# PABannier/bark.cpp

Hardware: NVIDIA H100
Metric: audio sec/sec (inverse RTF), bark-small f16, batch 1 per GPU, semantic->coarse->fine->encodec (higher is better)
Workload: dtype f16 weights/operands, f32 accumulate (reference arithmetic)

## Files before the change

bark.cpp_b200/csrc/bark_api.cu:

```cuda
#include "../../include/bark_b200.h"
#include "context.h"
#include "codec_kernels.h"
#include "gpt_kernels.h"

#include <algorithm>
#include <cmath>
#include <cstring>
#include <stdexcept>

using namespace bark;

namespace {

thread_local int g_device_override = -1;
bool quiet() { static const bool q = [] { const char * e = getenv("BARK_B200_QUIET"); return e && *e && *e != '0'; }(); return q; }

inline bool is_alpha(unsigned char c) { return (c >= 'a' && c <= 'z') || (c >= 'A' && c <= 'Z'); }
inline bool is_digit(unsigned char c) { return c >= '0' && c <= '9'; }
inline bool is_punct(unsigned char c) { return c > 32 && c < 127 && !is_alpha(c) && !is_digit(c); }

char fold_accent(unsigned char second) {
    const unsigned cp = 0xC0u + (second - 0x80u);
    const bool lower = cp >= 0xE0;
    const unsigned up = lower ? cp - 0x20 : cp;
// ... 626 lines not shown
}

extern "C" struct bark_context * bark_load_model(const char * model_path, struct bark_context_params params, uint32_t seed) {
    const int64_t t0 = now_us();
    if (!model_path) { fprintf(stderr, "%s: null model path\n", __func__); return nullptr; }
    cudaDeviceProp prop;
    const int dev = select_device(__func__, &prop);
    if (dev < 0) return nullptr;
    bark_context * ctx = new bark_context();
    ctx->device = dev;
    ctx->n_sm = ctx->n_sm_total = prop.multiProcessorCount;
    if (ctx->n_sm >= 132) ctx->n_sm = 128;
    { const char * e = getenv("BARK_B200_MODE"); ctx->fast_mode = e && !strcmp(e, "fast"); }
    { const char * e = getenv("BARK_B200_DECODE_CTAS"); if (e && atoi(e) >= 64 && atoi(e) <= ctx->n_sm) ctx->n_sm = atoi(e); }
    { const char * e = getenv("BARK_B200_SAMPLE_FLAG_EVERY"); ctx->debug_flag_every = e ? atoi(e) : 0; }
    { const char * e = getenv("BARK_B200_KV_REUSE"); ctx->kv_reuse = !(e && !strcmp(e, "0")); }
    { const char * e = getenv("BARK_B200_DECODE"); ctx->use_decode_kernel = !(e && !strcmp(e, "multi")); }
    { const char * e = getenv("BARK_B200_DECODE_TIMING_TID"); if (e && atoi(e) >= 0 && atoi(e) < 512) ctx->timing_tid = atoi(e) & ~31; }
    { const char * e = getenv("BARK_B200_POLL_NS"); if (e && atoi(e) >= 0 && atoi(e) <= 100000) ctx->poll_ns = (unsigned) atoi(e); }
    { const char * e = getenv("BARK_B200_HEADSTART"); if (e) { unsigned v[6]; if (sscanf(e, "%u:%u:%u:%u:%u:%u", &v[0], &v[1], &v[2], &v[3], &v[4], &v[5]) == 6) for (int i = 0; i < 6; i++) ctx->headstart[i] = std::min(v[i], 100000u); } }
    ctx->params = params;
    const bool loaded = guarded(false, [&] {
    BARK_CUDA_CHECK(cudaStreamCreateWithFlags(&ctx->stream, cudaStreamNonBlocking));
    if (!load_model_file(model_path, ctx)) return false;
    alloc_workspace(ctx);
    { const char * e = getenv("BARK_B200_TAG_BASE"); if (e) ctx->tag_base = (unsigned) strtoul(e, nullptr, 0); }
    if (getenv("BARK_B200_DECODE_TIMING")) { ctx->d_timing = (unsigned long long *) ctx_alloc(ctx, 256 * 32 * 8); BARK_CUDA_CHECK(cudaMemset(ctx->d_timing, 0, 256 * 32 * 8)); }
    BARK_CUDA_CHECK(cudaStreamSynchronize(ctx->stream));
    return true;
    });
// ... 262 lines not shown
```

bark.cpp_b200/csrc/common.cuh:

```cuda
#pragma once

#include <cuda_fp16.h>
#include <cuda_runtime.h>
#include <atomic>
#include <exception>
#include <stdexcept>
#include <stdint.h>
#include <stdio.h>
#include <stdlib.h>

namespace bark { struct CudaFailure { cudaError_t err; const char * file; int line; }; }
#define BARK_CUDA_CHECK(expr)                                                                         \
    do {                                                                                              \
        cudaError_t err__ = (expr);                                                                   \
        if (err__ != cudaSuccess) {                                                                   \
            fprintf(stderr, "bark_b200: CUDA error %s at %s:%d: %s\n", cudaGetErrorName(err__), __FILE__, __LINE__, \
                    cudaGetErrorString(err__));                                                       \
            throw ::bark::CudaFailure{err__, __FILE__, __LINE__};                                     \
        }                                                                                             \
    } while (0)

namespace bark {

template <typename R, typename F> inline R guarded(R fail, F && f) {
// ... 1 lines not shown
    catch (const CudaFailure &) { return fail; }
    catch (const std::exception & e) { fprintf(stderr, "bark_b200: %s\n", e.what()); return fail; }
    catch (...) { fprintf(stderr, "bark_b200: unexpected exception\n"); return fail; }
}

extern std::atomic<unsigned long long> g_kernel_launches;
extern std::atomic<unsigned long long> g_h2d_bytes, g_d2h_bytes;
inline bool first_use_on_this_device(std::atomic<unsigned long long> & mask) {
    int dev = 0;
    if (cudaGetDevice(&dev) != cudaSuccess || dev < 0 || dev > 63) return true;
    return !(mask.fetch_or(1ull << dev) >> dev & 1ull);
}
extern bool g_prof_on;
void prof_begin(const char * name, cudaStream_t s, double bytes, double flops);
void prof_end(cudaStream_t s);
extern thread_local double g_next_bytes, g_next_flops;
#define BARK_LAUNCH(kernel, grid, block, smem, stream, ...)                                           \
    do {                                                                                              \
        if (::bark::g_prof_on) ::bark::prof_begin(#kernel, (stream), ::bark::g_next_bytes, ::bark::g_next_flops);            \
        kernel<<<(grid), (block), (smem), (stream)>>>(__VA_ARGS__);                                   \
        if (::bark::g_prof_on) ::bark::prof_end((stream));                                            \
        ::bark::g_next_bytes = ::bark::g_next_flops = 0.0;                                                                    \
        ++::bark::g_kernel_launches;                                                                  \
    } while (0)

#define BARK_LAUNCH_PDL(kernel, grid, block, smem, strm__, ...)                                       \
    do {                                                                                              \
        if (::bark::g_prof_on) ::bark::prof_begin(#kernel, (strm__), ::bark::g_next_bytes, ::bark::g_next_flops);            \
        cudaLaunchConfig_t cfg__ = {};                                                                \
        cfg__.gridDim = (grid); cfg__.blockDim = (block); cfg__.dynamicSmemBytes = (smem); cfg__.stream = (strm__);          \
// ... 194 lines not shown
```

bark.cpp_b200/csrc/context.h:

```cpp
#pragma once
#include "../../include/bark_b200.h"
#include "gpt_kernels.h"

#include <fstream>
#include <map>
#include <random>
#include <string>
#include <vector>

struct ShardState {
    bool on = false; int rank = 0, world = 1;
    unsigned char * local = nullptr, * peer[8] = {nullptr};
    unsigned epoch = 0; unsigned * d_err = nullptr;
    unsigned long long nvlink_bytes = 0;
};

struct HistoryPrompt {
    std::vector<int32_t> semantic;
    std::vector<int32_t> coarse;
    std::vector<int32_t> fine;
    bool empty() const { return semantic.empty(); }
};

struct Generation {
// ... 15 lines not shown
};

struct bark_context {
    int device = 0;
    cudaStream_t stream = nullptr;

    bark::GPTModel semantic, coarse, fine;
    bark::CodecModel codec;
    std::map<std::string, int32_t> token_to_id;

    __half * d_gelu_tab = nullptr;
    unsigned * d_ln_fallbacks = nullptr;
    unsigned tag_base = 0;
    int n_sm = 0, n_sm_total = 0; bool use_decode_kernel = true;
    bool kv_reuse = true; unsigned long long n_kv_reused = 0;
    unsigned headstart[6] = {0, 2000, 500, 400, 500, 0};
    int timing_tid = 0; unsigned poll_ns = 40;
    unsigned long long * d_timing = nullptr;

    bool fast_mode = false;
    __half * f_a16 = nullptr, * f_h16 = nullptr, * f_qk16 = nullptr, * f_vt16 = nullptr, * f_att16 = nullptr;

    ShardState shard;

    bark::Workspace ws;
    bark::Q8Scratch q8;
    const float * last_logits = nullptr;
    double * d_u = nullptr, * h_u = nullptr;
    int32_t * d_stok = nullptr, * h_stok = nullptr, * d_sflags = nullptr, * h_sflags = nullptr;
    float * d_seos = nullptr, * h_seos = nullptr;
// ... 24 lines not shown

bool gpt_eval(bark_context * ctx, GPTModel & m, const int32_t * tokens, int n, int * n_past, bool merge_ctx, float * logits_host, int lm_lo = 0, int lm_hi = 0,
              float * mem_k = nullptr, float * mem_v = nullptr);
bool gpt_step_batch(bark_context * ctx, GPTModel & m, int B, float * const * slot_k, float * const * slot_v, const int32_t * tokens, const int * n_past,
                    int lm_lo, int lm_hi, float * d_logits);
void build_decode_tables(bark_context * ctx, GPTModel & m);
bool fine_eval(bark_context * ctx, const int32_t * in_buffer , int nn, float * logits_host );
bool fine_eval_shard(bark_context * ctx, const int32_t * in_buffer, int nn);
bool sample_shard(bark_context * ctx, std::mt19937 & rng, int n, float temp, int32_t * out_all );
bool fine_eval_fast(bark_context * ctx, const int32_t * in_buffer, int nn, float * logits_host);
bool gpt_decode_chained(bark_context * ctx, GPTModel & m, const int32_t * d_token, int * n_past, int lm_lo, int lm_hi);
bool fine_embed(bark_context * ctx, const int32_t * in_buffer, int nn, int row0, int rows, const char * fn);
void output_head(bark_context * ctx, const GPTModel & m, const float * x, int rows, const DMat & head, float * logits, int lo = 0);

struct ActLayout { WType wt; int kpE, kp4E; };
template <class KV> void run_layers(bark_context * ctx, const GPTModel & m, int rows, const KV & kv);
struct ShardKV {
    int row0;
    void store(bark_context * ctx, const GPTModel & m, int il, int rows, MatmulEpilogue & qkv) const;
    void attend(bark_context * ctx, const GPTModel & m, int il, int rows, const ActLayout & a) const;
};
bool load_codec(std::ifstream & f, CodecModel & c, int max_q, DeviceArena & arena, cudaStream_t s, bool verbose);
constexpr int kCodecLaunchFrames = 24000;
bool codec_decode(const CodecModel & cm, CodecScratch & sc, cudaStream_t s, int n, const int32_t * const * codes, const int * T, int n_q,
                  std::vector<float> * audio, const char * batch_fn = nullptr);
struct CodecOutputs { std::vector<int32_t> * codes = nullptr; std::vector<float> * latent = nullptr, * audio = nullptr; };
constexpr int kCodecSampleRate = 24000;
struct AudioFormat { int channels, sample_rate; };
bool codec_encode(const CodecModel & cm, CodecScratch & sc, cudaStream_t s, int n, const float * const * audio, const int * n_samples, int n_q,
                  const CodecOutputs & out, const char * batch_fn = nullptr, const AudioFormat * fmt = nullptr);
bool resample_input_ok(const char * fn, const std::string & item, const float * x, int n_frames, int channels, int sample_rate);
// ... 22 lines not shown
```

bark.cpp_b200/csrc/gemm_kernels.cu:

```cuda
#include "epilogue.cuh"
#include "gpt_kernels.h"

#include <algorithm>
#include <string.h>

namespace bark {

namespace {

__device__ __forceinline__ uint32_t smem_u32(const void * p) { return (uint32_t) __cvta_generic_to_shared(p); }
__device__ __forceinline__ void mbar_init(uint32_t bar, uint32_t count) { asm volatile("mbarrier.init.shared::cta.b64 [%0], %1;" ::"r"(bar), "r"(count)); }
__device__ __forceinline__ void mbar_expect_tx(uint32_t bar, uint32_t bytes) { asm volatile("mbarrier.arrive.expect_tx.shared::cta.b64 _, [%0], %1;" ::"r"(bar), "r"(bytes) : "memory"); }
__device__ __forceinline__ void mbar_wait(uint32_t bar, uint32_t parity) {
    asm volatile(
        "{\n\t.reg .pred p;\n\t"
        "WAIT_%=:\n\t"
        "mbarrier.try_wait.parity.shared::cta.b64 p, [%0], %1;\n\t"
        "@p bra DONE_%=;\n\t"
        "bra WAIT_%=;\n\t"
        "DONE_%=:\n\t}" ::"r"(bar), "r"(parity) : "memory");
}
__device__ __forceinline__ int atom_add_acq_rel_cta(int * p, int v) {
    int old;
    asm volatile("atom.acq_rel.cta.shared::cta.add.u32 %0, [%1], %2;" : "=r"(old) : "r"(smem_u32(p)), "r"(v) : "memory");
// ... 9 lines not shown
    for (int i = 0; i < N / 2; i++) {
        const float keep = upper ? r[i + N / 2] : r[i];
        const float send = upper ? r[i] : r[i + N / 2];
        r[i] = __fadd_rn(keep, __shfl_xor_sync(0xffffffffu, send, MASK));
    }
}
__device__ __forceinline__ int butterfly_reduce64(float (&r)[64], int lane) {
    butterfly_stage<64, 16>(r, (lane & 16) != 0);
    butterfly_stage<32, 8>(r, (lane & 8) != 0);
    butterfly_stage<16, 4>(r, (lane & 4) != 0);
    butterfly_stage<8, 1>(r, (lane & 1) != 0);
    butterfly_stage<4, 2>(r, (lane & 2) != 0);
    return ((lane & 16) << 1) | ((lane & 8) << 1) | ((lane & 4) << 1) | ((lane & 1) << 2) | (lane & 2);
}

constexpr int kStages = 4;
constexpr int kRedLd = 36;

template <int WM_, int WO_, int OT_, int MINB_, bool PIPE_ = false> struct TileCfg {
    static constexpr int WM = WM_, WO = WO_, OT = OT_, MINB = MINB_;
    static constexpr bool PIPE = PIPE_;
    static constexpr int kWarps = WM * WO, kThreads = 32 * kWarps, kBM = 8 * WM, kBO = OT * WO, kNAcc = 8 * OT;
    static constexpr int kStageBytes = (kBM + kBO) * 512;
    static constexpr bool kSmemReduce = MINB == 1;
    static constexpr size_t kRedOff = ((size_t) kStages * kStageBytes + kStages * 12 + 15) & ~(size_t) 15;
    static constexpr size_t kSmem = kRedOff + (kSmemReduce ? (size_t) kWarps * 32 * kRedLd * 4 : 0);
};
typedef TileCfg<4, 2, 8, 2>  Tile32x16;
typedef TileCfg<4, 4, 8, 1, true> Tile32x32;

template <typename T> struct QuadOp;
template <> struct QuadOp<__half> {
    typedef uint2 V;
    static constexpr int kGroupsPerStage = 2;
    __device__ __forceinline__ static float elem(const uint2 & u, int c) {
        const uint32_t w = c < 2 ? u.x : u.y;
        const __half2 h = *reinterpret_cast<const __half2 *>(&w);
        return (c & 1) ? __high2float(h) : __low2float(h);
    }
};
template <> struct QuadOp<float> {
    typedef uint4 V;
    static constexpr int kGroupsPerStage = 1;
    __device__ __forceinline__ static float elem(const uint4 & u, int c) { return __uint_as_float(c == 0 ? u.x : c == 1 ? u.y : c == 2 ? u.z : u.w); }
// ... 38 lines not shown
#pragma unroll
            for (int oi = 0; oi < OT; oi++) acc[mi * OT + oi] = __fmaf_rn(wf[oi], af[mi], acc[mi * OT + oi]);
    }
}
template <int OT>
__device__ __forceinline__ void load_half(const unsigned char * ga, const unsigned char * gw, int h, uint32_t (&a)[8], uint32_t (&w)[OT]) {
#pragma unroll
    for (int mi = 0; mi < 8; mi++) a[mi] = *reinterpret_cast<const uint32_t *>(ga + mi * 256 + h * 4);
#pragma unroll
    for (int oi = 0; oi < OT; oi++) w[oi] = *reinterpret_cast<const uint32_t *>(gw + oi * 256 + h * 4);
}

}

template <typename T, typename Cfg>
__global__ void __launch_bounds__(Cfg::kThreads, Cfg::MINB) lane_gemm_tiled_kernel(const T * __restrict__ Wg, int K, int w_gs, int O, const T * __restrict__ act, int act_gs, int M, MatmulEpilogue ep) {
    constexpr int GPS = QuadOp<T>::kGroupsPerStage, OT = Cfg::OT, kBM = Cfg::kBM, kBO = Cfg::kBO, kStageBytes = Cfg::kStageBytes;
    constexpr int kRowB = kGmGroup * sizeof(T);
    extern __shared__ __align__(128) unsigned char smem[];
    const uint32_t full = smem_u32(smem + kStages * kStageBytes);
    int * const cnt = reinterpret_cast<int *>(smem + kStages * kStageBytes + kStages * 8);
    const int tid = threadIdx.x, lane = tid & 31, warp = tid >> 5;
    const int wm = warp / Cfg::WO, wo = warp % Cfg::WO;
    const int nsteps = K >> 5;
    const int ngroups = (nsteps + 3) >> 2;
    const int nstages = (ngroups + GPS - 1) / GPS;
    const int tiles_o = (O + kBO - 1) / kBO, tiles_m = (M + kBM - 1) / kBM, n_tiles = tiles_o * tiles_m;
    const int my_tiles = ((int) blockIdx.x < n_tiles) ? (n_tiles - 1 - (int) blockIdx.x) / (int) gridDim.x + 1 : 0;
    const int total_steps = my_tiles * nstages;

    if (tid == 0) {
        for (int s = 0; s < kStages; s++) { mbar_init(full + s * 8, 1); cnt[s] = 0; }
// ... 45 lines not shown
                }
            }
#pragma unroll
            for (int j = 0; j < GPS; j++) {
                const int g = sg * GPS + j;
                if (g < ngroups) {
                    const unsigned char * ga = ga0 + j * (kBM + kBO) * kRowB, * gw = gw0 + j * (kBM + kBO) * kRowB;
                    const int steps = nsteps - g * 4;
                    if (steps >= 4) fma_group<T, OT, true>(ga, gw, acc, 4);
                    else            fma_group<T, OT, false>(ga, gw, acc, steps);
                }
            }
        released:
            __syncwarp();
            if (lane == 0) {
                if ((atom_add_acq_rel_cta(&cnt[slot], 1) + 1) % Cfg::kWarps == 0) {
                    asm volatile("fence.proxy.async.shared::cta;" ::: "memory");
                    if (step + kStages < total_steps) issue(step + kStages);
                }
            }
        }
        if constexpr (Cfg::kSmemReduce) {
            float * const red = reinterpret_cast<float *>(smem + Cfg::kRedOff) + warp * 32 * kRedLd;
#pragma unroll
            for (int sl = 0; sl < Cfg::kNAcc / 32; sl++) {
                __syncwarp();
#pragma unroll
                for (int j = 0; j < 32; j++) red[j * kRedLd + lane] = acc[sl * 32 + j];
                __syncwarp();
                float a[32];
#pragma unroll
                for (int q = 0; q < 8; q++) {
                    const float4 t = *reinterpret_cast<const float4 *>(red + lane * kRedLd + q * 4);
                    a[4 * q] = t.x; a[4 * q + 1] = t.y; a[4 * q + 2] = t.z; a[4 * q + 3] = t.w;
                }
                const int i = sl * 32 + lane;
                const int m = m0 + wm * 8 + i / OT, o = o0 + wo * OT + i % OT;
                const float r = lane_tree_reduce_local(a);
                if (m < M && o < O) matmul_epilogue(ep, m, o, r);
            }
        } else {
            static_assert(Cfg::kNAcc == 64, "the butterfly combines 64 outputs");
            const int base = butterfly_reduce64(acc, lane);
            const int m = m0 + wm * 8 + (base >> 3), o = o0 + wo * 8 + (base & 7);
            if (m < M) {
                if (o < O) matmul_epilogue(ep, m, o, acc[0]);
                if (o + 1 < O) matmul_epilogue(ep, m, o + 1, acc[1]);
            }
        }
    }
}

template <typename T, typename Cfg>
static void launch_tiled(const DMat & W, const void * act, int act_gs, int rows, const MatmulEpilogue & ep, int n_sm, cudaStream_t s) {
    static std::atomic<unsigned long long> configured{0};
    if (first_use_on_this_device(configured))
        BARK_CUDA_CHECK(cudaFuncSetAttribute(lane_gemm_tiled_kernel<T, Cfg>, cudaFuncAttributeMaxDynamicSharedMemorySize, (int) Cfg::kSmem));
    const int n_tiles = ((W.n_out + Cfg::kBO - 1) / Cfg::kBO) * ((rows + Cfg::kBM - 1) / Cfg::kBM);
    const int grid = min(n_tiles, Cfg::MINB * n_sm);
    BARK_LAUNCH((lane_gemm_tiled_kernel<T, Cfg>), grid, Cfg::kThreads, Cfg::kSmem, s, (const T *) W.p_gm, W.K, W.o_pad * kGmGroup, W.n_out,
                (const T *) act, act_gs, rows, ep);
}

int lane_gemm_tiled(const DMat & W, const void * act, int act_gs, int rows, const MatmulEpilogue & ep, cudaStream_t s, int variant) {
    if (!W.p_gm) { fprintf(stderr, "bark_b200: matrix has no group-major copy for the tiled mat-mul\n"); throw std::runtime_error("unsupported configuration (see the message above)"); }
    if (W.o_pad % kGemmOPad) { fprintf(stderr, "bark_b200: group-major rows padded to %d, need a multiple of %d\n", W.o_pad, kGemmOPad); throw std::runtime_error("unsupported configuration (see the message above)"); }
    int dev = 0, n_sm = 0;
    BARK_CUDA_CHECK(cudaGetDevice(&dev));
    BARK_CUDA_CHECK(cudaDeviceGetAttribute(&n_sm, cudaDevAttrMultiProcessorCount, dev));
    if (variant == 0) variant = W.type == W_F16 ? 2 : 1;
    if (W.type == W_F16) {
        if (variant == 1) launch_tiled<__half, Tile32x16>(W, act, act_gs, rows, ep, n_sm, s);
        else if (variant == 2) launch_tiled<__half, Tile32x32>(W, act, act_gs, rows, ep, n_sm, s);
        else return 0;
    } else if (W.type == W_F32) {
        if (variant == 1) launch_tiled<float, Tile32x16>(W, act, act_gs, rows, ep, n_sm, s);
        else return 0;
    } else return 0;
    return variant;
}

constexpr int kAttnQ = 32, kAttnKT = 64, kAttnVK = 512, kAttnVW = 16;
constexpr int kAttnVLd = kAttnVW + 4;

__host__ __device__ inline int attn_ld(int n_kv) { return ((n_kv + 31) & ~31) + 1; }
__host__ __device__ inline int attn_ring_off(int n_kv) { return (kAttnQ * attn_ld(n_kv) + 3) & ~3; }

namespace {
// ... 263 lines not shown
```

bark.cpp_b200/csrc/gpt_forward.cu:

```cuda
#include "context.h"
#include "gpt_kernels.h"

#include <algorithm>
#include <vector>
#include <time.h>

namespace bark {

int64_t now_us() {
    timespec ts; clock_gettime(CLOCK_MONOTONIC, &ts);
    return (int64_t) ts.tv_sec * 1000000 + ts.tv_nsec / 1000;
}


static ActLayout act_layout(const Workspace & ws, const GPTModel & m) {
    if (is_quant(m.wtype)) return {W_Q4_0, m.n_embd, 4 * m.n_embd};
    return {m.wtype, ws.max_rows * kGmGroup, ws.max_rows * kGmGroup};
}

template <class KV> void run_layers(bark_context * ctx, const GPTModel & m, int rows, const KV & kv) {
    Workspace & ws = ctx->ws;
    cudaStream_t s = ctx->stream;
    const int E = m.n_embd;
    const ActLayout a = act_layout(ws, m);
    for (int il = 0; il < m.n_layer; il++) {
        const GPTLayer & L = m.layers[(size_t) il];
        layernorm_act(ws.x, rows, E, L.ln_1_g, L.ln_1_b, ws.act, a.wt, a.kpE, ctx->d_ln_fallbacks, s);
        MatmulEpilogue qkv; qkv.mode = EPI_QKV; qkv.out = ws.q; qkv.ldo = E;
        kv.store(ctx, m, il, rows, qkv);
        lane_matmul(L.c_attn, ws.act, a.kpE, rows, qkv, &ctx->q8, s);
        kv.attend(ctx, m, il, rows, a);
        MatmulEpilogue res; res.mode = EPI_RESID; res.out = ws.x; res.ldo = E;
        lane_matmul(L.c_proj, ws.act, a.kpE, rows, res, &ctx->q8, s);
        layernorm_act(ws.x, rows, E, L.ln_2_g, L.ln_2_b, ws.act, a.wt, a.kpE, ctx->d_ln_fallbacks, s);
        MatmulEpilogue ge; ge.mode = EPI_GELU_ACT; ge.act_out = ws.act2; ge.act_wt = (int) a.wt; ge.act_Kp = a.kp4E; ge.gelu_tab = ctx->d_gelu_tab;
        lane_matmul(L.fc, ws.act, a.kpE, rows, ge, &ctx->q8, s);
        lane_matmul(L.proj, ws.act2, a.kp4E, rows, res, &ctx->q8, s);
    }
}
template void run_layers(bark_context *, const GPTModel &, int, const ShardKV &);

struct LocalKV {
    float * k, * v; size_t layer_floats; int n_past; bool causal;
    void store(bark_context *, const GPTModel & m, int il, int, MatmulEpilogue & qkv) const {
        const size_t at = il * layer_floats + (size_t) n_past * m.n_embd;
        qkv.k_out = k + at; qkv.v_out = v + at;
    }
    void attend(bark_context * ctx, const GPTModel & m, int il, int rows, const ActLayout & a) const {
        Workspace & ws = ctx->ws;
        attention(ws.q, k + il * layer_floats, v + il * layer_floats, rows, n_past + rows, n_past, m.n_embd, m.n_head, causal, ws.scores, ws.act, a.wt,
                  a.kpE, ctx->stream);
    }
};

struct SlotKV {
    float * const * slot_k, * const * slot_v; const int32_t * d_pos; int max_kv;
    void store(bark_context * ctx, const GPTModel &, int, int, MatmulEpilogue & qkv) const { qkv.k_out = ctx->ws.kbuf; qkv.v_out = ctx->ws.vbuf; }
    void attend(bark_context * ctx, const GPTModel & m, int il, int rows, const ActLayout & a) const {
        Workspace & ws = ctx->ws;
        const size_t layer = (size_t) il * m.block_size * m.n_embd;
        BatchKV kv;
        for (int b = 0; b < rows; b++) { kv.k[b] = slot_k[b] + layer; kv.v[b] = slot_v[b] + layer; }
        attention_batch(ws.q, ws.kbuf, ws.vbuf, kv, d_pos, rows, max_kv, m.n_embd, m.n_head, ws.scores, ws.act, a.wt, a.kpE, ctx->stream);
    }
};

void output_head(bark_context * ctx, const GPTModel & m, const float * x, int rows, const DMat & head, float * logits, int lo) {
    const ActLayout a = act_layout(ctx->ws, m);
// ... 87 lines not shown
              float * mem_k, float * mem_v) {
    if (!n_past) { fprintf(stderr, "%s: n_past is null\n", __func__); return false; }
    if (!mem_k || !mem_v) { mem_k = m.mem_k; mem_v = m.mem_v; }
    const int64_t t0 = now_us();
    Workspace & ws = ctx->ws;
    cudaStream_t s = ctx->stream;
    const int E = m.n_embd;
    int N = n;
    bool merge = false;
    clamp_lm(m, lm_lo, lm_hi);
    if (!tokens || n < 1 || n > 8 * 1024) { fprintf(stderr, "%s: bad token buffer (n = %d)\n", __func__, n); return false; }
    for (int i = 0; i < n; i++) if (tokens[i] < 0 || tokens[i] >= m.n_in_vocab) {
        fprintf(stderr, "%s: token id %d at position %d is outside the model's input vocabulary (%d)\n", __func__, tokens[i], i, m.n_in_vocab); return false;
    }
    if (*n_past > 0 && N == 1) {
        if (ctx->use_decode_kernel && m.decode_ok && *n_past + 1 <= m.block_size) {
            decode_step(ctx, m, tokens[0], nullptr, n_past, lm_lo, lm_hi, mem_k, mem_v);
            read_logits(ctx, m.glogits, lm_lo, lm_hi - lm_lo, logits_host);
            m.t_predict_us += now_us() - t0;
            return true;
        }
    } else if (merge_ctx && *n_past == 0) {
        if (N != 513) { fprintf(stderr, "%s: merged prompt must hold 256+256+1 ids (got %d)\n", __func__, N); return false; }
        N = 257; merge = true;
    }
    if (N < 1 || *n_past + N > m.block_size) { fprintf(stderr, "%s: context overflow (n_past %d + %d > %d)\n", __func__, *n_past, N, m.block_size); return false; }
    memcpy(ctx->h_tok, tokens, (size_t) n * sizeof(int32_t));
    BARK_CUDA_CHECK(cudaMemcpyAsync(ws.tok, ctx->h_tok, (size_t) n * sizeof(int32_t), cudaMemcpyHostToDevice, s)); g_h2d_bytes += (size_t) n * sizeof(int32_t);
    gpt_embed_causal(m, ws.tok, N, *n_past, merge, ws.x, s);
    run_layers(ctx, m, N, LocalKV{mem_k, mem_v, (size_t) m.block_size * E, *n_past, true});
    output_head(ctx, m, ws.x + (size_t)(N - 1) * E, 1, m.lm_head[0], ws.logits);
    read_logits(ctx, ws.logits, 0, m.n_out_vocab, logits_host);
    *n_past += N;
    m.t_predict_us += now_us() - t0;
    return true;
}

static DMat output_rows(const DMat & W, int lo, int hi) {
    DMat d = W;
    d.n_out = hi - lo; d.p_gm = nullptr; d.p_rm = nullptr;
    const size_t nb = (size_t) W.K / 32, r = (size_t) lo;
    auto at = [](void * p, size_t bytes) { return p ? (void *)((unsigned char *) p + bytes) : nullptr; };
    if (W.type == W_F16 || W.type == W_F32) { d.p = at(W.p, r * W.Kp * (W.type == W_F16 ? 2 : 4)); return d; }
    d.p = at(W.p, r * nb * (W.type == W_Q8_0 ? 32 : 16));
    d.scales = at(W.scales, r * nb * 2); d.mins = at(W.mins, r * nb * 2); d.qh = at(W.qh, r * nb * 4);
// ... 17 lines not shown
    }
    int32_t * h = ctx->batch.h_step, * d = ctx->batch.d_step;
    for (int b = 0; b < B; b++) { h[b] = tokens[b]; h[8 + b] = n_past[b]; }
    BARK_CUDA_CHECK(cudaMemcpyAsync(d, h, 16 * sizeof(int32_t), cudaMemcpyHostToDevice, s)); g_h2d_bytes += 16 * sizeof(int32_t);
    gpt_embed_causal(m, d, B, 0, false, ws.x, s, d + 8);
    run_layers(ctx, m, B, SlotKV{slot_k, slot_v, d + 8, max_kv});
    output_head(ctx, m, ws.x, B, output_rows(m.lm_head[0], lm_lo, lm_hi), d_logits, lm_lo);
    m.t_predict_us += now_us() - t0;
    return true;
}

bool gpt_decode_chained(bark_context * ctx, GPTModel & m, const int32_t * d_token, int * n_past, int lm_lo, int lm_hi) {
    if (!ctx->use_decode_kernel || !m.decode_ok || *n_past < 1) { fprintf(stderr, "%s: needs the persistent decode kernel and a filled KV cache\n", __func__); return false; }
    if (*n_past + 1 > m.block_size) { fprintf(stderr, "%s: context overflow (n_past %d + 1 > %d)\n", __func__, *n_past, m.block_size); return false; }
    clamp_lm(m, lm_lo, lm_hi);
    decode_step(ctx, m, 0, d_token, n_past, lm_lo, lm_hi, m.mem_k, m.mem_v);
    return true;
}

bool fine_embed(bark_context * ctx, const int32_t * in_buffer, int nn, int row0, int rows, const char * fn) {
    const GPTModel & m = ctx->fine;
    Workspace & ws = ctx->ws;
    if (nn < 1 || nn > 7) { fprintf(stderr, "%s: codebook index %d out of range\n", fn, nn); return false; }
    for (int i = 0; i < (nn + 1) * 1024; i++) if (in_buffer[i] < 0 || in_buffer[i] >= m.n_in_vocab) {
        fprintf(stderr, "%s: code %d (codebook %d, frame %d) is outside the fine model's input vocabulary (%d)\n", fn, in_buffer[i], i / 1024, i % 1024, m.n_in_vocab); return false;
    }
    memcpy(ctx->h_tok, in_buffer, (size_t) 8 * 1024 * sizeof(int32_t));
    BARK_CUDA_CHECK(cudaMemcpyAsync(ws.tok, ctx->h_tok, (size_t) 8 * 1024 * sizeof(int32_t), cudaMemcpyHostToDevice, ctx->stream)); g_h2d_bytes += (size_t) 8 * 1024 * sizeof(int32_t);
    gpt_embed_fine(m, ws.tok, nn, ws.x, ctx->stream, row0, rows);
    return true;
}

bool fine_eval(bark_context * ctx, const int32_t * in_buffer, int nn, float * logits_host) {
    if (ctx->fast_mode) return fine_eval_fast(ctx, in_buffer, nn, logits_host);
    GPTModel & m = ctx->fine;
    Workspace & ws = ctx->ws;
    const int64_t t0 = now_us();
    if (!fine_embed(ctx, in_buffer, nn, 0, 1024, __func__)) return false;
    run_layers(ctx, m, 1024, LocalKV{ws.kbuf, ws.vbuf, 0, 0, false});
    output_head(ctx, m, ws.x, 1024, m.lm_head[nn - 1], ws.logits);
    read_logits(ctx, ws.logits, 0, (size_t) 1024 * m.n_out_vocab, logits_host);
    m.t_predict_us += now_us() - t0;
    return true;
}

bool fine_eval_fast(bark_context * ctx, const int32_t * in_buffer, int nn, float * logits_host) {
    GPTModel & m = ctx->fine;
    const int64_t t0 = now_us();
    Workspace & ws = ctx->ws;
    cudaStream_t s = ctx->stream;
    const int E = m.n_embd, H = m.n_head, N = 1024, n_sm = ctx->n_sm_total;
    if (!fine_embed(ctx, in_buffer, nn, 0, N, __func__)) return false;
// ... 24 lines not shown
```

bark.cpp_b200/csrc/gpt_kernels.cu:

```cuda
#include "gpt_kernels.h"
#include "epilogue.cuh"

#include <cstring>

namespace bark {

std::atomic<unsigned long long> g_kernel_launches{0};

template <typename T>
__global__ void permute_to_li_kernel(const T * __restrict__ src, T * __restrict__ dst, int n_out, int K, int Kp) {
    constexpr int G = 16 / sizeof(T);
    const size_t total = (size_t) n_out * Kp;
    for (size_t i = (size_t) blockIdx.x * blockDim.x + threadIdx.x; i < total; i += (size_t) gridDim.x * blockDim.x) {
        const int o = (int)(i / Kp), j = (int)(i % Kp);
        const int e = j % G, gv = j / G, v = gv % 32, g = gv / 32;
        const int k = (g * G + e) * 32 + v;
        dst[i] = (k < K) ? src[(size_t) o * K + k] : T(0);
    }
}

void permute_to_li(const void * src, void * dst, int n_out, int K, WType t, cudaStream_t s) {
    if (t == W_F16) { const int Kp = li_padded_k(K, 2); BARK_LAUNCH(permute_to_li_kernel<__half>, 1184, 256, 0, s, (const __half *) src, (__half *) dst, n_out, K, Kp); }
    else            { const int Kp = li_padded_k(K, 4); BARK_LAUNCH(permute_to_li_kernel<float>, 1184, 256, 0, s, (const float *) src, (float *) dst, n_out, K, Kp); }
}
// ... 156 lines not shown
    for (int mi = 0; mi < MT; mi++) {
        const float r = lane_tree_reduce(acc[mi]);
        if (lane == 0 && mi < mvalid) matmul_epilogue(ep, m0 + mi, o, r);
    }
}

void lane_matmul(const DMat & W, const void * act, int act_gs, int rows, const MatmulEpilogue & ep, const Q8Scratch * q8, cudaStream_t s) {
    if (W.type == W_Q4_0) { q4_matmul(W, act, act_gs, rows, ep, q8, s); return; }
    if (qx_supported(W.type)) { qx_matmul(W, act, act_gs, rows, ep, q8, s); return; }
    const int gx = (W.n_out + 7) / 8;
    {
        const double es = W.type == W_F16 ? 2.0 : 4.0;
        g_next_bytes = (double) W.n_out * W.K * es + (double) rows * (W.K * es + W.n_out * 4.0);
        g_next_flops = 2.0 * rows * (double) W.n_out * W.K;
    }
    if (rows >= 16 && (W.type == W_F16 || W.type == W_F32)) { lane_gemm_tiled(W, act, act_gs, rows, ep, s); return; }
    if (W.type == W_F16) {
        if (rows == 1) BARK_LAUNCH((lane_matmul_kernel<__half, 1>), dim3(gx, 1), 256, 0, s, (const __half *) W.p, W.K, W.Kp, W.n_out, (const __half *) act, act_gs, rows, ep);
        else           BARK_LAUNCH((lane_matmul_kernel<__half, 8>), dim3(gx, (rows + 7) / 8), 256, 0, s, (const __half *) W.p, W.K, W.Kp, W.n_out, (const __half *) act, act_gs, rows, ep);
    } else if (W.type == W_F32) {
        if (rows == 1) BARK_LAUNCH((lane_matmul_kernel<float, 1>), dim3(gx, 1), 256, 0, s, (const float *) W.p, W.K, W.Kp, W.n_out, (const float *) act, act_gs, rows, ep);
        else           BARK_LAUNCH((lane_matmul_kernel<float, 8>), dim3(gx, (rows + 7) / 8), 256, 0, s, (const float *) W.p, W.K, W.Kp, W.n_out, (const float *) act, act_gs, rows, ep);
    } else {
        fprintf(stderr, "bark_b200: q4_0 mul_mat is not built in this revision\n"); throw std::runtime_error("unsupported configuration (see the message above)");
    }
}

__device__ __forceinline__ float * row_cache(float * const (&p)[8], int b) {
    float * r = p[0];
#pragma unroll
    for (int i = 1; i < 8; i++) if (b == i) r = p[i];
// ... 89 lines not shown
```

bark.cpp_b200/csrc/gpt_kernels.h:

```cpp
#pragma once
#include "model.h"

namespace bark {

enum EpiMode : int { EPI_STORE = 0, EPI_RESID = 1, EPI_GELU_ACT = 2, EPI_QKV = 3 };

struct MatmulEpilogue {
    int mode = EPI_STORE;
    float * out = nullptr; int ldo = 0;
    float * k_out = nullptr, * v_out = nullptr;
    int n_peer = 0; float * k_peer[7] = {nullptr}, * v_peer[7] = {nullptr};
    void * act_out = nullptr; int act_wt = 0, act_Kp = 0;
    const __half * gelu_tab = nullptr;
};

void permute_to_li(const void * src_rowmajor, void * dst_li, int n_out, int K, WType t, cudaStream_t s);
void permute_to_gm(const void * src_rowmajor, void * dst_gm, int n_out, int o_pad, int K, WType t, cudaStream_t s);

void gpt_embed_causal(const GPTModel & m, const int32_t * d_tok, int N, int n_past, bool merge, float * x, cudaStream_t s, const int32_t * d_pos = nullptr);
void gpt_embed_fine(const GPTModel & m, const int32_t * d_ids, int nn, float * x, cudaStream_t s, int row0 = 0, int rows = 1024);

void layernorm_act(const float * x, int rows, int E, const float * g, const float * b, void * act, WType wt, int Kp,
                   unsigned * fallback_counter, cudaStream_t s);

// ... 12 lines not shown
                     float * scores, void * act, WType wt, int Kp, cudaStream_t s);

void q4_split(const void * raw_blocks, size_t n_blocks, void * qs, void * scales, cudaStream_t s);
void q4_matmul(const DMat & W, const void * act_f32, int ld_act, int rows, const MatmulEpilogue & ep, const Q8Scratch * q8, cudaStream_t s);

bool   qx_supported(WType t);
size_t qx_block_bytes(WType t);
void   qx_split(const void * raw_blocks, size_t n_blocks, WType t, void * qs, void * qh, void * d, void * m, cudaStream_t s);
void   quantize_q8(const float * x, int ldx, int rows, int K, int8_t * q, float * d, float * s, cudaStream_t stream);
void   qx_embed_causal(const GPTModel & m, const int32_t * d_tok, int N, int n_past, bool merge, float * x, cudaStream_t s, const int32_t * d_pos);
void   qx_embed_fine(const GPTModel & m, const int32_t * d_ids, int nn, float * x, cudaStream_t s);
void   qx_matmul(const DMat & W, const void * act_f32, int ld_act, int rows, const MatmulEpilogue & ep, const Q8Scratch * q8, cudaStream_t s);

constexpr int kGemmOPad = 32;
int lane_gemm_tiled(const DMat & W, const void * act, int act_gs, int rows, const MatmulEpilogue & ep, cudaStream_t s, int variant = 0);

enum { FEPI_F32 = 0, FEPI_RESID = 1, FEPI_GELU16 = 2, FEPI_QKV16 = 4 };
struct FastEpi {
    int mode = FEPI_F32;
    float * out32 = nullptr; __half * out16 = nullptr; int ldo = 0;
    __half * vt = nullptr; int vt_ld = 0, v_col0 = 0;
};
int  fast_gemm(const __half * A, int lda, const __half * W, int ldw, int M, int N, int K, const FastEpi & ep, int n_sm, int bn, cudaStream_t s);
bool fast_attention(const __half * qk, int ldq, int k_col0, const __half * vt, int n, int E, int H, __half * out, cudaStream_t s);
void fast_layernorm(const float * x, int rows, int E, const float * g, const float * b, __half * out, cudaStream_t s);
void fast_convert(const void * src, WType t, int n_out, int K, __half * dst, int * non_finite, cudaStream_t s);

constexpr int kDecodeReplicas = 8;
struct DecodePhase { const void * w; int n_out, row_bytes, K, pad; const void * ws; };
struct DecodeLayerVec { const float * ln_1_g, * ln_1_b, * ln_2_g, * ln_2_b; };
// ... 23 lines not shown
```

bark.cpp_b200/csrc/prof.cu:

```cuda
#include "../../include/bark_b200.h"
#include "common.cuh"

#include <map>
#include <mutex>
#include <string>
#include <vector>

namespace bark {

std::atomic<unsigned long long> g_h2d_bytes{0}, g_d2h_bytes{0};
bool g_prof_on = false;
thread_local double g_next_bytes = 0.0, g_next_flops = 0.0;

namespace {
struct Rec { const char * name; cudaEvent_t a, b; double bytes, flops; };
std::vector<Rec> g_recs;
std::vector<cudaEvent_t> g_pool;
std::mutex g_prof_mutex;
cudaEvent_t get_event() {
    if (!g_pool.empty()) { cudaEvent_t e = g_pool.back(); g_pool.pop_back(); return e; }
    cudaEvent_t e; BARK_CUDA_CHECK(cudaEventCreate(&e)); return e;
}
}

void prof_begin(const char * name, cudaStream_t s, double bytes, double flops) {
    std::lock_guard<std::mutex> lock(g_prof_mutex);
    Rec r{name, get_event(), get_event(), bytes, flops};
    BARK_CUDA_CHECK(cudaEventRecord(r.a, s));
    g_recs.push_back(r);
}
void prof_end(cudaStream_t s) { std::lock_guard<std::mutex> lock(g_prof_mutex); BARK_CUDA_CHECK(cudaEventRecord(g_recs.back().b, s)); }

}

using namespace bark;

extern "C" void bark_b200_profile_enable(int on) {
    g_prof_on = on != 0;
    for (auto & r : g_recs) { g_pool.push_back(r.a); g_pool.push_back(r.b); }
    g_recs.clear();
}

static int bark_b200_profile_report_impl(char * buf, int cap) {
    BARK_CUDA_CHECK(cudaDeviceSynchronize());
    struct Agg { long n = 0; double ms = 0, bytes = 0, flops = 0; };
    std::map<std::string, Agg> agg;
    for (auto & r : g_recs) {
        float ms = 0; BARK_CUDA_CHECK(cudaEventElapsedTime(&ms, r.a, r.b));
        std::string n = r.name;
        if (!n.empty() && n.front() == '(') n = n.substr(1, n.size() - 2);
        Agg & a = agg[n]; a.n++; a.ms += ms; a.bytes += r.bytes; a.flops += r.flops;
    }
    std::string out = "{";
    bool first = true;
    for (auto & kv : agg) {
        char tmp[512];
        snprintf(tmp, sizeof tmp, "%s\"%s\": {\"launches\": %ld, \"ms\": %.6f, \"bytes\": %.6e, \"flops\": %.6e}", first ? "" : ", ", kv.first.c_str(), kv.second.n, kv.second.ms, kv.second.bytes, kv.second.flops);
        out += tmp; first = false;
    }
    out += "}";
    if (buf && cap > 0) { snprintf(buf, (size_t) cap, "%s", out.c_str()); }
    return (int) out.size() + 1;
}
extern "C" int bark_b200_profile_report(char * buf, int cap) { return guarded((int) 0, [&] { return bark_b200_profile_report_impl(buf, cap); }); }

// ... 6 lines not shown
```

Before: 12.79.

## Skip non-final rows in last layer of prompt passes and add few-row GEMM tile

For causal prompt forward passes, the last transformer layer now computes the attention output, projection and MLP only for the final row, since only that row's logits are used (BARK_B200_ALL_ROWS=1 restores full computation). The KV cache for all rows is still filled, because it is written by the QKV matmul. Separately, a new tiled GEMM variant whose block height matches the row count is selected for f16 matrices with at most 128 rows when the output tiles fit in the SM count, aiming at better SM fill for small-batch prompt GEMMs. Per-pass profiling labels are also added. Risks: the new tile uses fewer pipeline stages and no shared-memory reduction, and it checks the SM count on every call.

After: 12.87 (median of 6 runs). About the same (+0.6%).

```diff
diff --git a/bark.cpp_b200/csrc/bark_api.cu b/bark.cpp_b200/csrc/bark_api.cu
--- a/bark.cpp_b200/csrc/bark_api.cu
+++ b/bark.cpp_b200/csrc/bark_api.cu
@@ -664,6 +664,7 @@
     { const char * e = getenv("BARK_B200_MODE"); ctx->fast_mode = e && !strcmp(e, "fast"); }
     { const char * e = getenv("BARK_B200_DECODE_CTAS"); if (e && atoi(e) >= 64 && atoi(e) <= ctx->n_sm) ctx->n_sm = atoi(e); }
     { const char * e = getenv("BARK_B200_SAMPLE_FLAG_EVERY"); ctx->debug_flag_every = e ? atoi(e) : 0; }
+    { const char * e = getenv("BARK_B200_ALL_ROWS"); ctx->all_rows = e && !strcmp(e, "1"); }
     { const char * e = getenv("BARK_B200_KV_REUSE"); ctx->kv_reuse = !(e && !strcmp(e, "0")); }
     { const char * e = getenv("BARK_B200_DECODE"); ctx->use_decode_kernel = !(e && !strcmp(e, "multi")); }
     { const char * e = getenv("BARK_B200_DECODE_TIMING_TID"); if (e && atoi(e) >= 0 && atoi(e) < 512) ctx->timing_tid = atoi(e) & ~31; }
diff --git a/bark.cpp_b200/csrc/common.cuh b/bark.cpp_b200/csrc/common.cuh
--- a/bark.cpp_b200/csrc/common.cuh
+++ b/bark.cpp_b200/csrc/common.cuh
@@ -39,6 +39,12 @@
 extern bool g_prof_on;
 void prof_begin(const char * name, cudaStream_t s, double bytes, double flops);
 void prof_end(cudaStream_t s);
+extern thread_local const char * g_prof_pass;
+struct ProfPass {
+    const char * prev;
+    explicit ProfPass(const char * pass) : prev(g_prof_pass) { g_prof_pass = pass; }
+    ~ProfPass() { g_prof_pass = prev; }
+};
 extern thread_local double g_next_bytes, g_next_flops;
 #define BARK_LAUNCH(kernel, grid, block, smem, stream, ...)                                           \
     do {                                                                                              \
diff --git a/bark.cpp_b200/csrc/context.h b/bark.cpp_b200/csrc/context.h
--- a/bark.cpp_b200/csrc/context.h
+++ b/bark.cpp_b200/csrc/context.h
@@ -53,6 +53,7 @@
     unsigned tag_base = 0;
     int n_sm = 0, n_sm_total = 0; bool use_decode_kernel = true;
     bool kv_reuse = true; unsigned long long n_kv_reused = 0;
+    bool all_rows = false;
     unsigned headstart[6] = {0, 2000, 500, 400, 500, 0};
     int timing_tid = 0; unsigned poll_ns = 40;
     unsigned long long * d_timing = nullptr;
@@ -107,7 +108,7 @@
 void output_head(bark_context * ctx, const GPTModel & m, const float * x, int rows, const DMat & head, float * logits, int lo = 0);
 
 struct ActLayout { WType wt; int kpE, kp4E; };
-template <class KV> void run_layers(bark_context * ctx, const GPTModel & m, int rows, const KV & kv);
+template <class KV> void run_layers(bark_context * ctx, const GPTModel & m, int rows, const KV & kv, int last_rows = 0);
 struct ShardKV {
     int row0;
     void store(bark_context * ctx, const GPTModel & m, int il, int rows, MatmulEpilogue & qkv) const;
diff --git a/bark.cpp_b200/csrc/gemm_kernels.cu b/bark.cpp_b200/csrc/gemm_kernels.cu
--- a/bark.cpp_b200/csrc/gemm_kernels.cu
+++ b/bark.cpp_b200/csrc/gemm_kernels.cu
@@ -47,20 +47,25 @@
     return ((lane & 16) << 1) | ((lane & 8) << 1) | ((lane & 4) << 1) | ((lane & 1) << 2) | (lane & 2);
 }
 
-constexpr int kStages = 4;
 constexpr int kRedLd = 36;
 
-template <int WM_, int WO_, int OT_, int MINB_, bool PIPE_ = false> struct TileCfg {
+template <int WM_, int WO_, int OT_, int MINB_, bool PIPE_ = false, bool ALL_ROWS_ = false> struct TileCfg {
     static constexpr int WM = WM_, WO = WO_, OT = OT_, MINB = MINB_;
-    static constexpr bool PIPE = PIPE_;
+    static constexpr bool PIPE = PIPE_, ALL_ROWS = ALL_ROWS_;
     static constexpr int kWarps = WM * WO, kThreads = 32 * kWarps, kBM = 8 * WM, kBO = OT * WO, kNAcc = 8 * OT;
-    static constexpr int kStageBytes = (kBM + kBO) * 512;
-    static constexpr bool kSmemReduce = MINB == 1;
-    static constexpr size_t kRedOff = ((size_t) kStages * kStageBytes + kStages * 12 + 15) & ~(size_t) 15;
-    static constexpr size_t kSmem = kRedOff + (kSmemReduce ? (size_t) kWarps * 32 * kRedLd * 4 : 0);
+    static constexpr int kStages = ALL_ROWS ? 3 : 4;
+    __host__ __device__ static constexpr int bm(int M) { return ALL_ROWS ? (M + 7) & ~7 : kBM; }
+    __host__ __device__ static constexpr int warps(int M) { return bm(M) / 8 * WO; }
+    __host__ __device__ static constexpr int stage_bytes(int M) { return (bm(M) + kBO) * 512; }
+    static constexpr bool kSmemReduce = MINB == 1 && !ALL_ROWS;
+    __host__ __device__ static constexpr size_t red_off(int M) { return ((size_t) kStages * stage_bytes(M) + kStages * 12 + 15) & ~(size_t) 15; }
+    static constexpr size_t smem(int M) { return red_off(M) + (kSmemReduce ? (size_t) kWarps * 32 * kRedLd * 4 : 0); }
+    static constexpr size_t kSmem = smem(kBM);
 };
 typedef TileCfg<4, 2, 8, 2>  Tile32x16;
 typedef TileCfg<4, 4, 8, 1, true> Tile32x32;
+typedef TileCfg<16, 1, 8, 1, true, true> TileRowsx8;
+static_assert(TileRowsx8::kSmem <= 227 * 1024, "the few-row tile's ring must fit in shared memory at 128 rows");
 
 template <typename T> struct QuadOp;
 template <> struct QuadOp<__half> {
@@ -129,8 +134,9 @@
 }
 
 template <typename T, typename Cfg>
-__global__ void __launch_bounds__(Cfg::kThreads, Cfg::MINB) lane_gemm_tiled_kernel(const T * __restrict__ Wg, int K, int w_gs, int O, const T * __restrict__ act, int act_gs, int M, MatmulEpilogue ep) {
-    constexpr int GPS = QuadOp<T>::kGroupsPerStage, OT = Cfg::OT, kBM = Cfg::kBM, kBO = Cfg::kBO, kStageBytes = Cfg::kStageBytes;
+__device__ __forceinline__ void lane_gemm_tiled_body(const T * __restrict__ Wg, int K, int w_gs, int O, const T * __restrict__ act, int act_gs, int M, const MatmulEpilogue & ep) {
+    constexpr int GPS = QuadOp<T>::kGroupsPerStage, OT = Cfg::OT, kBO = Cfg::kBO, kStages = Cfg::kStages;
+    const int kBM = Cfg::bm(M), kStageBytes = Cfg::stage_bytes(M), n_warps = Cfg::warps(M);
     constexpr int kRowB = kGmGroup * sizeof(T);
     extern __shared__ __align__(128) unsigned char smem[];
     const uint32_t full = smem_u32(smem + kStages * kStageBytes);
@@ -206,14 +212,14 @@
         released:
             __syncwarp();
             if (lane == 0) {
-                if ((atom_add_acq_rel_cta(&cnt[slot], 1) + 1) % Cfg::kWarps == 0) {
+                if ((atom_add_acq_rel_cta(&cnt[slot], 1) + 1) % n_warps == 0) {
                     asm volatile("fence.proxy.async.shared::cta;" ::: "memory");
                     if (step + kStages < total_steps) issue(step + kStages);
                 }
             }
         }
         if constexpr (Cfg::kSmemReduce) {
-            float * const red = reinterpret_cast<float *>(smem + Cfg::kRedOff) + warp * 32 * kRedLd;
+            float * const red = reinterpret_cast<float *>(smem + Cfg::red_off(M)) + warp * 32 * kRedLd;
 #pragma unroll
             for (int sl = 0; sl < Cfg::kNAcc / 32; sl++) {
                 __syncwarp();
@@ -244,26 +250,52 @@
 }
 
 template <typename T, typename Cfg>
+__global__ void __launch_bounds__(Cfg::kThreads, Cfg::MINB) lane_gemm_tiled_kernel(const T * __restrict__ Wg, int K, int w_gs, int O, const T * __restrict__ act, int act_gs, int M, MatmulEpilogue ep) {
+    lane_gemm_tiled_body<T, Cfg>(Wg, K, w_gs, O, act, act_gs, M, ep);
+}
+template <typename T, typename Cfg>
+__global__ void __launch_bounds__(Cfg::kThreads, Cfg::MINB) lane_gemm_rows_kernel(const T * __restrict__ Wg, int K, int w_gs, int O, const T * __restrict__ act, int act_gs, int M, MatmulEpilogue ep) {
+    lane_gemm_tiled_body<T, Cfg>(Wg, K, w_gs, O, act, act_gs, M, ep);
+}
+
+template <typename T, typename Cfg>
 static void launch_tiled(const DMat & W, const void * act, int act_gs, int rows, const MatmulEpilogue & ep, int n_sm, cudaStream_t s) {
     static std::atomic<unsigned long long> configured{0};
-    if (first_use_on_this_device(configured))
-        BARK_CUDA_CHECK(cudaFuncSetAttribute(lane_gemm_tiled_kernel<T, Cfg>, cudaFuncAttributeMaxDynamicSharedMemorySize, (int) Cfg::kSmem));
-    const int n_tiles = ((W.n_out + Cfg::kBO - 1) / Cfg::kBO) * ((rows + Cfg::kBM - 1) / Cfg::kBM);
+    const int n_tiles = ((W.n_out + Cfg::kBO - 1) / Cfg::kBO) * ((rows + Cfg::bm(rows) - 1) / Cfg::bm(rows));
     const int grid = min(n_tiles, Cfg::MINB * n_sm);
-    BARK_LAUNCH((lane_gemm_tiled_kernel<T, Cfg>), grid, Cfg::kThreads, Cfg::kSmem, s, (const T *) W.p_gm, W.K, W.o_pad * kGmGroup, W.n_out,
-                (const T *) act, act_gs, rows, ep);
+    if constexpr (Cfg::ALL_ROWS) {
+        if (first_use_on_this_device(configured))
+            BARK_CUDA_CHECK(cudaFuncSetAttribute(lane_gemm_rows_kernel<T, Cfg>, cudaFuncAttributeMaxDynamicSharedMemorySize, (int) Cfg::kSmem));
+        BARK_LAUNCH((lane_gemm_rows_kernel<T, Cfg>), grid, 32 * Cfg::warps(rows), Cfg::smem(rows), s, (const T *) W.p_gm, W.K, W.o_pad * kGmGroup, W.n_out,
+                    (const T *) act, act_gs, rows, ep);
+    } else {
+        if (first_use_on_this_device(configured))
+            BARK_CUDA_CHECK(cudaFuncSetAttribute(lane_gemm_tiled_kernel<T, Cfg>, cudaFuncAttributeMaxDynamicSharedMemorySize, (int) Cfg::kSmem));
+        BARK_LAUNCH((lane_gemm_tiled_kernel<T, Cfg>), grid, 32 * Cfg::warps(rows), Cfg::smem(rows), s, (const T *) W.p_gm, W.K, W.o_pad * kGmGroup, W.n_out,
+                    (const T *) act, act_gs, rows, ep);
+    }
+}
+
+static int sm_count_now() {
+    int dev = 0, n_sm = 0;
+    BARK_CUDA_CHECK(cudaGetDevice(&dev));
+    BARK_CUDA_CHECK(cudaDeviceGetAttribute(&n_sm, cudaDevAttrMultiProcessorCount, dev));
+    return n_sm;
+}
+
+bool gemm_few_rows(const DMat & W, int rows) {
+    return W.type == W_F16 && rows <= TileRowsx8::kBM && (W.n_out + TileRowsx8::kBO - 1) / TileRowsx8::kBO <= sm_count_now();
 }
 
 int lane_gemm_tiled(const DMat & W, const void * act, int act_gs, int rows, const MatmulEpilogue & ep, cudaStream_t s, int variant) {
     if (!W.p_gm) { fprintf(stderr, "bark_b200: matrix has no group-major copy for the tiled mat-mul\n"); throw std::runtime_error("unsupported configuration (see the message above)"); }
     if (W.o_pad % kGemmOPad) { fprintf(stderr, "bark_b200: group-major rows padded to %d, need a multiple of %d\n", W.o_pad, kGemmOPad); throw std::runtime_error("unsupported configuration (see the message above)"); }
-    int dev = 0, n_sm = 0;
-    BARK_CUDA_CHECK(cudaGetDevice(&dev));
-    BARK_CUDA_CHECK(cudaDeviceGetAttribute(&n_sm, cudaDevAttrMultiProcessorCount, dev));
+    const int n_sm = sm_count_now();
     if (variant == 0) variant = W.type == W_F16 ? 2 : 1;
     if (W.type == W_F16) {
         if (variant == 1) launch_tiled<__half, Tile32x16>(W, act, act_gs, rows, ep, n_sm, s);
         else if (variant == 2) launch_tiled<__half, Tile32x32>(W, act, act_gs, rows, ep, n_sm, s);
+        else if (variant == 3 && rows <= TileRowsx8::kBM) launch_tiled<__half, TileRowsx8>(W, act, act_gs, rows, ep, n_sm, s);
         else return 0;
     } else if (W.type == W_F32) {
         if (variant == 1) launch_tiled<float, Tile32x16>(W, act, act_gs, rows, ep, n_sm, s);
diff --git a/bark.cpp_b200/csrc/gpt_forward.cu b/bark.cpp_b200/csrc/gpt_forward.cu
--- a/bark.cpp_b200/csrc/gpt_forward.cu
+++ b/bark.cpp_b200/csrc/gpt_forward.cu
@@ -2,6 +2,7 @@
 #include "gpt_kernels.h"
 
 #include <algorithm>
+#include <type_traits>
 #include <vector>
 #include <time.h>
 
@@ -18,7 +19,20 @@
     return {m.wtype, ws.max_rows * kGmGroup, ws.max_rows * kGmGroup};
 }
 
-template <class KV> void run_layers(bark_context * ctx, const GPTModel & m, int rows, const KV & kv) {
+struct LocalKV {
+    float * k, * v; size_t layer_floats; int n_past; bool causal;
+    void store(bark_context *, const GPTModel & m, int il, int, MatmulEpilogue & qkv) const {
+        const size_t at = il * layer_floats + (size_t) n_past * m.n_embd;
+        qkv.k_out = k + at; qkv.v_out = v + at;
+    }
+    void attend(bark_context * ctx, const GPTModel & m, int il, int rows, const ActLayout & a, int r0 = 0) const {
+        Workspace & ws = ctx->ws;
+        attention(ws.q + (size_t) r0 * m.n_embd, k + il * layer_floats, v + il * layer_floats, rows - r0, n_past + rows, n_past + r0, m.n_embd, m.n_head,
+                  causal, ws.scores, ws.act, a.wt, a.kpE, ctx->stream);
+    }
+};
+
+template <class KV> void run_layers(bark_context * ctx, const GPTModel & m, int rows, const KV & kv, int last_rows) {
     Workspace & ws = ctx->ws;
     cudaStream_t s = ctx->stream;
     const int E = m.n_embd;
@@ -29,29 +43,24 @@
         MatmulEpilogue qkv; qkv.mode = EPI_QKV; qkv.out = ws.q; qkv.ldo = E;
         kv.store(ctx, m, il, rows, qkv);
         lane_matmul(L.c_attn, ws.act, a.kpE, rows, qkv, &ctx->q8, s);
-        kv.attend(ctx, m, il, rows, a);
-        MatmulEpilogue res; res.mode = EPI_RESID; res.out = ws.x; res.ldo = E;
-        lane_matmul(L.c_proj, ws.act, a.kpE, rows, res, &ctx->q8, s);
-        layernorm_act(ws.x, rows, E, L.ln_2_g, L.ln_2_b, ws.act, a.wt, a.kpE, ctx->d_ln_fallbacks, s);
+        int r0 = 0;
+        if constexpr (std::is_same<KV, LocalKV>::value) {
+            if (il == m.n_layer - 1 && last_rows > 0 && last_rows < rows) r0 = rows - last_rows;
+            kv.attend(ctx, m, il, rows, a, r0);
+        } else {
+            kv.attend(ctx, m, il, rows, a);
+        }
+        float * const x = ws.x + (size_t) r0 * E;
+        const int n = rows - r0;
+        MatmulEpilogue res; res.mode = EPI_RESID; res.out = x; res.ldo = E;
+        lane_matmul(L.c_proj, ws.act, a.kpE, n, res, &ctx->q8, s);
+        layernorm_act(x, n, E, L.ln_2_g, L.ln_2_b, ws.act, a.wt, a.kpE, ctx->d_ln_fallbacks, s);
         MatmulEpilogue ge; ge.mode = EPI_GELU_ACT; ge.act_out = ws.act2; ge.act_wt = (int) a.wt; ge.act_Kp = a.kp4E; ge.gelu_tab = ctx->d_gelu_tab;
-        lane_matmul(L.fc, ws.act, a.kpE, rows, ge, &ctx->q8, s);
-        lane_matmul(L.proj, ws.act2, a.kp4E, rows, res, &ctx->q8, s);
-    }
-}
-template void run_layers(bark_context *, const GPTModel &, int, const ShardKV &);
-
-struct LocalKV {
-    float * k, * v; size_t layer_floats; int n_past; bool causal;
-    void store(bark_context *, const GPTModel & m, int il, int, MatmulEpilogue & qkv) const {
-        const size_t at = il * layer_floats + (size_t) n_past * m.n_embd;
-        qkv.k_out = k + at; qkv.v_out = v + at;
-    }
-    void attend(bark_context * ctx, const GPTModel & m, int il, int rows, const ActLayout & a) const {
-        Workspace & ws = ctx->ws;
-        attention(ws.q, k + il * layer_floats, v + il * layer_floats, rows, n_past + rows, n_past, m.n_embd, m.n_head, causal, ws.scores, ws.act, a.wt,
-                  a.kpE, ctx->stream);
-    }
-};
+        lane_matmul(L.fc, ws.act, a.kpE, n, ge, &ctx->q8, s);
+        lane_matmul(L.proj, ws.act2, a.kp4E, n, res, &ctx->q8, s);
+    }
+}
+template void run_layers(bark_context *, const GPTModel &, int, const ShardKV &, int);
 
 struct SlotKV {
     float * const * slot_k, * const * slot_v; const int32_t * d_pos; int max_kv;
@@ -169,6 +178,7 @@
         fprintf(stderr, "%s: token id %d at position %d is outside the model's input vocabulary (%d)\n", __func__, tokens[i], i, m.n_in_vocab); return false;
     }
     if (*n_past > 0 && N == 1) {
+        ProfPass pass("decode");
         if (ctx->use_decode_kernel && m.decode_ok && *n_past + 1 <= m.block_size) {
             decode_step(ctx, m, tokens[0], nullptr, n_past, lm_lo, lm_hi, mem_k, mem_v);
             read_logits(ctx, m.glogits, lm_lo, lm_hi - lm_lo, logits_host);
@@ -180,10 +190,11 @@
         N = 257; merge = true;
     }
     if (N < 1 || *n_past + N > m.block_size) { fprintf(stderr, "%s: context overflow (n_past %d + %d > %d)\n", __func__, *n_past, N, m.block_size); return false; }
+    ProfPass pass(N == 1 ? "decode" : &m == &ctx->semantic ? "semantic_prompt" : *n_past == 0 ? "coarse_first_window" : "coarse_later_window");
     memcpy(ctx->h_tok, tokens, (size_t) n * sizeof(int32_t));
     BARK_CUDA_CHECK(cudaMemcpyAsync(ws.tok, ctx->h_tok, (size_t) n * sizeof(int32_t), cudaMemcpyHostToDevice, s)); g_h2d_bytes += (size_t) n * sizeof(int32_t);
     gpt_embed_causal(m, ws.tok, N, *n_past, merge, ws.x, s);
-    run_layers(ctx, m, N, LocalKV{mem_k, mem_v, (size_t) m.block_size * E, *n_past, true});
+    run_layers(ctx, m, N, LocalKV{mem_k, mem_v, (size_t) m.block_size * E, *n_past, true}, ctx->all_rows ? N : 1);
     output_head(ctx, m, ws.x + (size_t)(N - 1) * E, 1, m.lm_head[0], ws.logits);
     read_logits(ctx, ws.logits, 0, m.n_out_vocab, logits_host);
     *n_past += N;
@@ -231,6 +242,7 @@
     if (!ctx->use_decode_kernel || !m.decode_ok || *n_past < 1) { fprintf(stderr, "%s: needs the persistent decode kernel and a filled KV cache\n", __func__); return false; }
     if (*n_past + 1 > m.block_size) { fprintf(stderr, "%s: context overflow (n_past %d + 1 > %d)\n", __func__, *n_past, m.block_size); return false; }
     clamp_lm(m, lm_lo, lm_hi);
+    ProfPass pass("decode");
     decode_step(ctx, m, 0, d_token, n_past, lm_lo, lm_hi, m.mem_k, m.mem_v);
     return true;
 }
@@ -253,6 +265,7 @@
     GPTModel & m = ctx->fine;
     Workspace & ws = ctx->ws;
     const int64_t t0 = now_us();
+    ProfPass pass("fine");
     if (!fine_embed(ctx, in_buffer, nn, 0, 1024, __func__)) return false;
     run_layers(ctx, m, 1024, LocalKV{ws.kbuf, ws.vbuf, 0, 0, false});
     output_head(ctx, m, ws.x, 1024, m.lm_head[nn - 1], ws.logits);
diff --git a/bark.cpp_b200/csrc/gpt_kernels.cu b/bark.cpp_b200/csrc/gpt_kernels.cu
--- a/bark.cpp_b200/csrc/gpt_kernels.cu
+++ b/bark.cpp_b200/csrc/gpt_kernels.cu
@@ -194,7 +194,7 @@
         g_next_bytes = (double) W.n_out * W.K * es + (double) rows * (W.K * es + W.n_out * 4.0);
         g_next_flops = 2.0 * rows * (double) W.n_out * W.K;
     }
-    if (rows >= 16 && (W.type == W_F16 || W.type == W_F32)) { lane_gemm_tiled(W, act, act_gs, rows, ep, s); return; }
+    if (rows >= 16 && (W.type == W_F16 || W.type == W_F32)) { lane_gemm_tiled(W, act, act_gs, rows, ep, s, gemm_few_rows(W, rows) ? 3 : 0); return; }
     if (W.type == W_F16) {
         if (rows == 1) BARK_LAUNCH((lane_matmul_kernel<__half, 1>), dim3(gx, 1), 256, 0, s, (const __half *) W.p, W.K, W.Kp, W.n_out, (const __half *) act, act_gs, rows, ep);
         else           BARK_LAUNCH((lane_matmul_kernel<__half, 8>), dim3(gx, (rows + 7) / 8), 256, 0, s, (const __half *) W.p, W.K, W.Kp, W.n_out, (const __half *) act, act_gs, rows, ep);
diff --git a/bark.cpp_b200/csrc/gpt_kernels.h b/bark.cpp_b200/csrc/gpt_kernels.h
--- a/bark.cpp_b200/csrc/gpt_kernels.h
+++ b/bark.cpp_b200/csrc/gpt_kernels.h
@@ -50,6 +50,7 @@
 
 constexpr int kGemmOPad = 32;
 int lane_gemm_tiled(const DMat & W, const void * act, int act_gs, int rows, const MatmulEpilogue & ep, cudaStream_t s, int variant = 0);
+bool gemm_few_rows(const DMat & W, int rows);
 
 enum { FEPI_F32 = 0, FEPI_RESID = 1, FEPI_GELU16 = 2, FEPI_QKV16 = 4 };
 struct FastEpi {
diff --git a/bark.cpp_b200/csrc/prof.cu b/bark.cpp_b200/csrc/prof.cu
--- a/bark.cpp_b200/csrc/prof.cu
+++ b/bark.cpp_b200/csrc/prof.cu
@@ -4,6 +4,7 @@
 #include <map>
 #include <mutex>
 #include <string>
+#include <string.h>
 #include <vector>
 
 namespace bark {
@@ -11,9 +12,11 @@
 std::atomic<unsigned long long> g_h2d_bytes{0}, g_d2h_bytes{0};
 bool g_prof_on = false;
 thread_local double g_next_bytes = 0.0, g_next_flops = 0.0;
+thread_local const char * g_prof_pass = nullptr;
 
 namespace {
-struct Rec { const char * name; cudaEvent_t a, b; double bytes, flops; };
+struct Rec { const char * name, * pass; cudaEvent_t a, b; double bytes, flops; };
+bool by_pass() { static const bool on = [] { const char * e = getenv("BARK_B200_PROFILE_PASSES"); return e && !strcmp(e, "1"); }(); return on; }
 std::vector<Rec> g_recs;
 std::vector<cudaEvent_t> g_pool;
 std::mutex g_prof_mutex;
@@ -25,7 +28,7 @@
 
 void prof_begin(const char * name, cudaStream_t s, double bytes, double flops) {
     std::lock_guard<std::mutex> lock(g_prof_mutex);
-    Rec r{name, get_event(), get_event(), bytes, flops};
+    Rec r{name, g_prof_pass ? g_prof_pass : "other", get_event(), get_event(), bytes, flops};
     BARK_CUDA_CHECK(cudaEventRecord(r.a, s));
     g_recs.push_back(r);
 }
@@ -49,6 +52,7 @@
         float ms = 0; BARK_CUDA_CHECK(cudaEventElapsedTime(&ms, r.a, r.b));
         std::string n = r.name;
         if (!n.empty() && n.front() == '(') n = n.substr(1, n.size() - 2);
+        if (by_pass()) n = std::string(r.pass) + "|" + n;
         Agg & a = agg[n]; a.n++; a.ms += ms; a.bytes += r.bytes; a.flops += r.flops;
     }
     std::string out = "{";
```
